# samukallio/path-tracer

Measured on AMD Instinct MI355X. Metric: Mrays/s + Msamples/s, Viking Room 1920x1080 1024spp, 1/2/4/8 GPUs, higher is better.
Workload: dtype f32; 1 GPU; C3 scene, one 1920x1080 1024-spp frame per step (Reset, Run(2), Run(1) until the frame's sample count reaches 1024 x pixels); each of 1 GPU(s) renders every pixel with its own RNG stream to 1/1 of the samples, then the reduce of radiance + sample counts to rank 0; spp_target=1024, streams=1, slots_per_launch_rank0=2073600, split=3, class_lists=False, frame_target_samples_rank0=2123366400, mesh_faces=3976, parallelism=sample-shards x1

## Files before the change

### include/pt_scene.h

```cpp
#ifndef PT_SCENE_H
#define PT_SCENE_H

#include <stdint.h>
#include "pt_packed.h"

#ifdef __cplusplus
extern "C" {
#endif

typedef struct pts_scene pts_scene;
typedef struct pts_entity pts_entity;
typedef struct pts_material pts_material;
typedef struct pts_texture pts_texture;
typedef struct pts_mesh pts_mesh;
typedef struct pts_prefab pts_prefab;

enum {
    PTS_ENTITY_ROOT = 0,
    PTS_ENTITY_CONTAINER = 1,
    PTS_ENTITY_CAMERA = 2,
    PTS_ENTITY_MESH_INSTANCE = 3,
    PTS_ENTITY_PLANE = 4,
    PTS_ENTITY_SPHERE = 5,
    PTS_ENTITY_CUBE = 6,
// ... 93 lines not shown
int  ptsSaveSpectrumTable(const char* path);
int  ptsLoadSpectrumTable(const char* path);
void ptsSetSpectrumTablePath(const char* path);

int  ptsDenoise(uint32_t width, uint32_t height, const float* accum_rgba, const pt_denoise_guide* guides,
                const pt_denoise_parameters* params, float* out_rgba);
int  ptsDenoisePair(uint32_t width, uint32_t height, const float* accum_a, const float* accum_b,
                    const pt_denoise_guide* guides, const pt_denoise_pair_parameters* params, float* out_rgba);

int  ptsReproject(uint32_t prev_width, uint32_t prev_height, const float* prev_accum,
                  const pt_denoise_guide* prev_guides, const pt_packed_camera* prev_camera, uint32_t width,
                  uint32_t height, const pt_denoise_guide* guides, const pt_packed_camera* camera,
                  const pt_reproject_parameters* params, float* out_rgba);
int  ptsShapeMotion(const pt_packed_shape* prev_shapes, uint32_t prev_count, const pt_packed_shape* shapes,
                    uint32_t count, pt_shape_motion* out);
int  ptsReprojectMoving(uint32_t prev_width, uint32_t prev_height, const float* prev_accum,
                        const pt_denoise_guide* prev_guides, const pt_packed_camera* prev_camera, uint32_t width,
                        uint32_t height, const pt_denoise_guide* guides, const pt_packed_camera* camera,
                        const pt_shape_motion* motion, uint32_t motion_count, const pt_reproject_parameters* params,
                        float* out_rgba);
int  ptsRectifyHistory(uint32_t width, uint32_t height, const float* history, const float* current,
                       const pt_denoise_guide* guides, const pt_rectify_parameters* params, float* out_rgba);
int  ptsDespike(uint32_t width, uint32_t height, const float* accum, const pt_denoise_guide* guides,
                const pt_despike_parameters* params, float* out_rgba);
int  ptsCentralCameraRay(const pt_packed_camera* camera, uint32_t x, uint32_t y, uint32_t width, uint32_t height,
                         float origin[3], float velocity[3]);
int  ptsAmbientOcclusionRays(const pt_ambient_occlusion_parameters* params, uint32_t x, uint32_t y,
                             const float origin[3], const float velocity[3], float time, const float normal[3],
                             float* out_origins, uint32_t* out_velocities, float* out_duration);
int  ptsGatherVisibilityRays(const pt_visibility_gather_parameters* params, uint32_t n, const float* points,
                             const float* normals, float* out_origins, uint32_t* out_velocities,
                             float* out_durations);
int  ptsGatherVisibilityReduce(uint32_t samples, uint32_t n, const uint32_t* packed, const uint64_t* occluded_bits,
                               pt_visibility_record* out);
uint32_t ptsVisibilitySkip(uint32_t state, uint32_t steps);
int  ptsSkyGatherRays(const pt_sky_gather_parameters* params, uint32_t n, const float* points, const float* normals,
                      float* out_origins, uint32_t* out_velocities, float* out_durations, float* out_lambda0);
int  ptsSkyGatherReduce(uint32_t samples, uint32_t n, const uint32_t* packed, const uint64_t* occluded_bits,
                        const float* contributions, pt_sky_record* out);
int  ptsSkyGatherBasis(uint32_t n, const uint32_t* packed, float* out);

int  ptsFrameStatistics(uint32_t width, uint32_t height, const float* accum_a, const float* accum_b,
                        pt_frame_statistics* out);
int  ptsTileStatistics(uint32_t width, uint32_t height, const float* accum_a, const float* accum_b,
                       float noise_threshold, pt_tile_statistics* out);
int    ptsStatsBin(float value);
double ptsStatsBinEdge(int bin);
int    ptsStatsPercentileBin(const uint32_t* histogram, double q);
double ptsStatsLogAverage(const uint32_t* histogram, double q_lo, double q_hi);
double ptsStatsAutoBrightness(const pt_frame_statistics* stats, double key, double q_lo, double q_hi);
double ptsStatsNoise(const pt_frame_statistics* stats, double q);
uint32_t ptsRayKey(const float origin[3], const float velocity[3], const float lo[3], const float hi[3]);

#ifdef __cplusplus
}
#endif

#endif
```

### path-tracer_amd/_native.py

```python
from __future__ import annotations

import ctypes as C
import os
from pathlib import Path

import numpy as np

PKG = Path(__file__).resolve().parent
SCENE_LIB_PATH = PKG / "libptscene.so"
HIP_LIB_PATH = PKG / "libpathtracer.so"


class NativeLibraryMissing(RuntimeError):
    pass



class pt_scene_packs(C.Structure):
    _fields_ = [
        ("globals", C.c_void_p),
        ("textures", C.c_void_p), ("texture_count", C.c_uint32),
        ("material_data", C.c_void_p), ("material_word_count", C.c_uint32),
        ("shapes", C.c_void_p), ("shape_count", C.c_uint32),
        ("shape_nodes", C.c_void_p), ("shape_node_count", C.c_uint32),
# ... 329 lines not shown
    "ptsDefaultLoadModelOptions": (None, [C.POINTER(pts_load_model_options)]),
    "ptsLoadTexture": (_vp, [_vp, C.c_char_p, _i32, C.c_char_p]),
    "ptsLoadImageRGBA8": (_i32, [C.c_char_p, C.POINTER(C.c_uint32), C.POINTER(C.c_uint32), _vp]),
    "ptsLoadModelAsPrefab": (_vp, [_vp, C.c_char_p, C.POINTER(pts_load_model_options)]),
    "ptsInstantiatePrefab": (_vp, [_vp, _vp, _vp]),
    "ptsLoadScene": (_vp, [C.c_char_p]),
    "ptsSaveScene": (_i32, [_vp, C.c_char_p]),
    "ptsSceneTextureCount": (_u32, [_vp]),
    "ptsSceneMaterialCount": (_u32, [_vp]),
    "ptsSceneMeshCount": (_u32, [_vp]),
    "ptsScenePrefabCount": (_u32, [_vp]),
    "ptsPrefabMeshCount": (_u32, [_vp]),
    "ptsPrefabMesh": (_vp, [_vp, _u32, C.POINTER(_vp), _fptr]),
    "ptsMeshVertexCount": (_u32, [_vp]),
    "ptsMeshFaceCount": (_u32, [_vp]),
    "ptsMeshVertices": (None, [_vp, _fptr]),
    "ptsMaterialType": (_i32, [_vp]),
    "ptsPackSceneData": (_u32, [_vp]),
    "ptsGetScenePacks": (None, [_vp, C.POINTER(pt_scene_packs)]),
    "ptsMarkDirty": (None, [_vp, _u32]),
    "ptsGetParametricSpectrumCoefficients": (_i32, [_fptr, _fptr]),
    "ptsBuildSpectrumTable": (_i32, [_i32]),
    "ptsSaveSpectrumTable": (_i32, [C.c_char_p]),
    "ptsLoadSpectrumTable": (_i32, [C.c_char_p]),
    "ptsSetSpectrumTablePath": (None, [C.c_char_p]),
    "ptsDenoise": (_i32, [_u32, _u32, _fptr, _vp, C.POINTER(pt_denoise_parameters), _fptr]),
    "ptsDenoisePair": (_i32, [_u32, _u32, _fptr, _fptr, _vp, C.POINTER(pt_denoise_pair_parameters), _fptr]),
    "ptsReproject": (_i32, [_u32, _u32, _fptr, _vp, C.POINTER(pt_packed_camera), _u32, _u32, _vp,
                            C.POINTER(pt_packed_camera), C.POINTER(pt_reproject_parameters), _fptr]),
    "ptsShapeMotion": (_i32, [_vp, _u32, _vp, _u32, _vp]),
    "ptsReprojectMoving": (_i32, [_u32, _u32, _fptr, _vp, C.POINTER(pt_packed_camera), _u32, _u32, _vp,
                                  C.POINTER(pt_packed_camera), _vp, _u32, C.POINTER(pt_reproject_parameters), _fptr]),
    "ptsRectifyHistory": (_i32, [_u32, _u32, _fptr, _fptr, _vp, C.POINTER(pt_rectify_parameters), _fptr]),
    "ptsDespike": (_i32, [_u32, _u32, _fptr, _vp, C.POINTER(pt_despike_parameters), _fptr]),
    "ptsCentralCameraRay": (_i32, [C.POINTER(pt_packed_camera), _u32, _u32, _u32, _u32, _fptr, _fptr]),
    "ptsAmbientOcclusionRays": (_i32, [C.POINTER(pt_ambient_occlusion_parameters), _u32, _u32, _fptr, _fptr, _f32,
                                       _fptr, _fptr, _u32ptr, _fptr]),
    "ptsGatherVisibilityRays": (_i32, [C.POINTER(pt_visibility_gather_parameters), _u32, _fptr, _fptr, _fptr, _u32ptr,
                                       _fptr]),
    "ptsGatherVisibilityReduce": (_i32, [_u32, _u32, _u32ptr, C.POINTER(C.c_uint64), _vp]),
    "ptsVisibilitySkip": (_u32, [_u32, _u32]),
    "ptsSkyGatherRays": (_i32, [C.POINTER(pt_sky_gather_parameters), _u32, _fptr, _fptr, _fptr, _u32ptr, _fptr, _fptr]),
    "ptsSkyGatherReduce": (_i32, [_u32, _u32, _u32ptr, C.POINTER(C.c_uint64), _fptr, _vp]),
    "ptsSkyGatherBasis": (_i32, [_u32, _u32ptr, _fptr]),
    "ptsFrameStatistics": (_i32, [_u32, _u32, _fptr, _fptr, C.POINTER(pt_frame_statistics)]),
    "ptsTileStatistics": (_i32, [_u32, _u32, _fptr, _fptr, _f32, _vp]),
    "ptsStatsBin": (_i32, [C.c_float]),
    "ptsStatsBinEdge": (C.c_double, [_i32]),
    "ptsStatsPercentileBin": (_i32, [_u32ptr, C.c_double]),
    "ptsStatsLogAverage": (C.c_double, [_u32ptr, C.c_double, C.c_double]),
    "ptsStatsAutoBrightness": (C.c_double, [C.POINTER(pt_frame_statistics), C.c_double, C.c_double, C.c_double]),
    "ptsStatsNoise": (C.c_double, [C.POINTER(pt_frame_statistics), C.c_double]),
    "ptsRayKey": (_u32, [_fptr, _fptr, _fptr, _fptr]),
}

HIP_API = {
    "ptGetLastError": (C.c_char_p, []),
    "ptGetDeviceCount": (_i32, [C.POINTER(_i32)]),
    "ptCreateDevice": (_vp, [_i32]),
    "ptDestroyDevice": (None, [_vp]),
    "ptSynchronize": (_i32, [_vp]),
    "ptCreateScene": (_vp, [_vp]),
    "ptUpdateScene": (_i32, [_vp, _vp, C.POINTER(pt_scene_packs), _u32]),
    "ptSetSceneStackFormat": (_i32, [_vp, _u32]),
    "ptSetSceneHitRecordForm": (_i32, [_vp, _u32]),
    "ptSetSceneExtendForm": (_i32, [_vp, _u32]),
    "ptGetSceneExtendForm": (_i32, [_vp, C.POINTER(C.c_uint32)]),
    "ptDestroyScene": (None, [_vp, _vp]),
    "ptCreateSampleBuffer": (_vp, [_vp, _u32, _u32]),
    "ptDestroySampleBuffer": (None, [_vp, _vp]),
    "ptReadSampleBuffer": (_i32, [_vp, _vp, _fptr]),
    "ptWriteSampleBuffer": (_i32, [_vp, _vp, _fptr]),
    "ptRenderSampleBuffer": (_i32, [_vp, _vp, C.POINTER(pt_resolve_parameters)]),
    "ptReadResolvedImage": (_i32, [_vp, _vp, _fptr]),
    "ptReadResolvedImageSRGB8": (_i32, [_vp, _vp, C.POINTER(C.c_uint8)]),
    "ptCreateBasicRenderer": (_vp, [_vp, _vp, _vp]),
    "ptCreateBasicRendererPartitioned": (_vp, [_vp, _vp, _vp, _u32, _u32]),
    "ptCreateBasicRendererStreams": (_vp, [_vp, _vp, _vp, _u32, _u32, _u32]),
    "ptMergeBasicRendererStreams": (_i32, [_vp, _vp]),
    "ptBasicRendererStreams": (_u32, [_vp]),
    "ptReadBasicRendererStreamState": (_i32, [_vp, _vp, _u32, _vp]),
    "ptWriteBasicRendererState": (_i32, [_vp, _vp, _vp]),
    "ptWriteBasicRendererStreamState": (_i32, [_vp, _vp, _u32, _vp]),
    "ptReadBasicRendererStreamAccumulator": (_i32, [_vp, _vp, _u32, _fptr]),
    "ptWriteBasicRendererStreamAccumulator": (_i32, [_vp, _vp, _u32, _fptr]),
    "ptGetBasicRendererShadeInfo": (_i32, [_vp, C.POINTER(pt_shade_info)]),
    "ptDestroyBasicRenderer": (None, [_vp, _vp]),
    "ptBasicRendererParams": (C.POINTER(pt_basic_renderer_params), [_vp]),
    "ptResetBasicRenderer": (_i32, [_vp, _vp]),
    "ptRunBasicRenderer": (_i32, [_vp, _vp, _u32]),
    "ptBasicRendererSlotCount": (_u32, [_vp]),
    "ptSetBasicRendererFusedRounds": (_i32, [_vp, _i32]),
    "ptRunBasicRendererRounds": (_i32, [_vp, _vp, _u32]),
    "ptSetBasicRendererRoundBatch": (_i32, [_vp, _u32]),
    "ptSetBasicRendererSplit": (_i32, [_vp, _u32]),
    "ptSetBasicRendererClassLists": (_i32, [_vp, _u32]),
    "ptGetBasicRendererClassLists": (_i32, [_vp, _u32ptr]),
    "ptGetBasicRendererSplit": (_i32, [_vp, _u32ptr, _u32ptr, _u32ptr]),
    "ptSetBasicRendererRayOrder": (_i32, [_vp, _u32]),
    "ptGetBasicRendererRayOrder": (_i32, [_vp, _u32ptr, _u32ptr]),
    "ptSetBasicRendererBlockMap": (_i32, [_vp, _u32]),
    "ptGetBasicRendererBlockMap": (_i32, [_vp, _u32ptr, _u32ptr]),
    "ptBlockMapGroupTileCount": (_u32, [_u32, _u32, _u32, _u32]),
    "ptBlockMapGroupTile": (_u32, [_u32, _u32, _u32, _u32, _u32]),
    "ptBlockMapGroupTileStart": (_u32, [_u32, _u32, _u32, _u32]),
    "ptBlockMapGroupUnitCount": (_u32, [_u32, _u32, _u32, _u32]),
# ... 119 lines not shown
```

### path-tracer_amd/csrc/hip/pt_device.hpp

```cpp
#pragma once

#include <hip/hip_runtime.h>
#include "../../../include/pt_glsl.h"
#include "../../../include/pt_packed.h"

#define PT_DEV __device__ __forceinline__

namespace ptd {

constexpr uint32_t SHAPE_INDEX_NONE = 0xFFFFFFFFu;
constexpr uint32_t TEXTURE_INDEX_NONE = 0xFFFFFFFFu;
constexpr uint32_t PT_SHAPE_FLAG_UV = 1u;

struct dscene {
    pt_packed_scene_globals g;
    const pt_packed_texture* textures;
    const uint32_t* material;
    const pt_packed_shape* shapes;
    const float4* shape_nodes;
    const float4* mesh_faces;
    const uint2* mesh_vertices;
    const float4* vertex_attr;
    const float* vertex_v;
    const float4* mesh_nodes;
    const pt_packed_camera* cameras;
    const float4* atlas;
    uint32_t atlas_w, atlas_h, atlas_layers;
    uint32_t atlas_tiled;
    uint32_t fast_div;
    uint32_t blas_words;
    uint32_t blas_firstbits;
    uint32_t stack16;
    uint32_t mat_classes;
    uint32_t vidx21;
    float vmf_inv_kappa, vmf_exp_m2k, vmf_norm;
    float sky_flat;
    uint32_t node_cache;
    uint32_t single_mesh;
    uint32_t mesh_root[2];
    float mesh_from[16];
};

#ifndef PT_NODE_CACHE_PAIRS
#define PT_NODE_CACHE_PAIRS 160
#endif

struct ray { pt3 Origin; pt3 Velocity; float Duration; };
struct medium { uint32_t Priority; pt4 IOR, AbsorptionRate, ScatteringRate; float ScatteringAnisotropy; };

PT_DEV pt3 xyz(float4 a) { return v3(a.x, a.y, a.z); }


PT_DEV pt3 TransformNormal(pt3 N, const float* From) { return normalize(vec_mul_mat4(N, From)); }
PT_DEV pt3 TransformDirection(pt3 D, const float* To) { return normalize(mat4_mul_vector(To, D)); }

PT_DEV pt3 SafeNormalize(pt3 V)
{
// ... 23 lines not shown
        float Sx = Px >= 0.0f ? 1.0f : -1.0f, Sy = Py >= 0.0f ? 1.0f : -1.0f;
        float Nx = (1.0f - pt_abs(Py)) * Sx;
        float Ny = (1.0f - pt_abs(Px)) * Sy;
        Px = Nx; Py = Ny;
    }
    return pt_pack_snorm16(Px) | (pt_pack_snorm16(Py) << 16);
}

PT_DEV pt3 UnpackUnitVector(uint32_t P)
{
    float Px = pt_unpack_snorm16(P & 0xFFFFu), Py = pt_unpack_snorm16(P >> 16);
    float Z = 1.0f - pt_abs(Px) - pt_abs(Py);
    if (Z < 0.0f) {
        float Sx = Px >= 0.0f ? 1.0f : -1.0f, Sy = Py >= 0.0f ? 1.0f : -1.0f;
        float Nx = (1.0f - pt_abs(Py)) * Sx;
        float Ny = (1.0f - pt_abs(Px)) * Sy;
        Px = Nx; Py = Ny;
    }
    return normalize(v3(Px, Py, Z));
}

PT_DEV float RecipForDiv(float b)
{
    float m = pt_abs(b);
    return (m >= 0x1p-100f && m <= 0x1p100f) ? 1.0f / b : pt_u2f(0x7fc00000u);
}

PT_DEV float XDiv(float a, float b, float y)
{
    float q = a * y;
    float r = __builtin_fmaf(-q, b, a);
    float q1 = __builtin_fmaf(r, y, q);
    float m = pt_abs(q1);
    if (!(m >= 0x1p-100f && m <= 0x1p100f && pt_abs(a) >= 0x1p-100f)) q1 = a / b;
    return q1;
}

PT_DEV float HwMin(float a, float b) { return __builtin_fminf(a, b); }
PT_DEV float HwMax(float a, float b) { return __builtin_fmaxf(a, b); }
PT_DEV float HwMin3(float a, float b, float c) { return __builtin_fminf(__builtin_fminf(a, b), c); }
PT_DEV float HwMax3(float a, float b, float c) { return __builtin_fmaxf(__builtin_fmaxf(a, b), c); }

PT_DEV float FastRcp(float d)
{
    float y = __builtin_amdgcn_rcpf(d);
    float e = __builtin_fmaf(-d, y, 1.0f);
    return __builtin_fmaf(e, y, y);
}


PT_DEV bool FastRcpRange(float d)
{
    float m = pt_abs(d);
    return (m >= 0x1p-126f) & (m < 0x1p126f);
}


PT_DEV bool FastDivRay(pt3 O, pt3 V)
{
    bool ok = true;
#define PT_CHECK_O(c) { float m = pt_abs(c); ok &= (m == 0.0f) | ((m >= 0x1p-50f) & (m <= 0x1p40f)); }
#define PT_CHECK_V(c) { float m = pt_abs(c); ok &= (m >= 0x1p-59f) & (m <= 0x1p27f); }
    PT_CHECK_O(O.x) PT_CHECK_O(O.y) PT_CHECK_O(O.z)
    PT_CHECK_V(V.x) PT_CHECK_V(V.y) PT_CHECK_V(V.z)
#undef PT_CHECK_O
#undef PT_CHECK_V
    return ok;
}

PT_DEV float FastQuot(float a, float b, float y)
{
    float q = a * y;
    float r = __builtin_fmaf(-q, b, a);
    return __builtin_fmaf(r, y, q);
}

PT_DEV float SlabEntry(float ax, float ay, float az, float bx, float by, float bz, float Reach)
{
    float EntryT = HwMax3(HwMin(ax, bx), HwMin(ay, by), HwMin(az, bz));
    float ExitT = HwMin3(HwMax(ax, bx), HwMax(ay, by), HwMax(az, bz));
    bool miss = (ExitT < EntryT) | (ExitT <= 0.0f) | (EntryT >= Reach);
    return miss ? PT_INFINITY : EntryT;
}

PT_DEV float IntersectBoundingBox(pt3 O, pt3 V, pt3 Y, float Reach, float4 MinAndX, float4 MaxAndX, bool exact)
{
    pt3 A = xyz(MinAndX) - O, B = xyz(MaxAndX) - O;
    if (exact)
        return SlabEntry(FastQuot(A.x, V.x, Y.x), FastQuot(A.y, V.y, Y.y), FastQuot(A.z, V.z, Y.z),
                         FastQuot(B.x, V.x, Y.x), FastQuot(B.y, V.y, Y.y), FastQuot(B.z, V.z, Y.z), Reach);
    return SlabEntry(A.x / V.x, A.y / V.y, A.z / V.z, B.x / V.x, B.y / V.y, B.z / V.z, Reach);
}

PT_DEV void IntersectBoxPair(pt3 O, pt3 V, pt3 Y, float Reach, float4 a0, float4 a1, float4 b0, float4 b1, bool exact,
                             float& TA, float& TB)
{
    if (exact) {
        TA = IntersectBoundingBox(O, V, Y, Reach, a0, a1, true);
        TB = IntersectBoundingBox(O, V, Y, Reach, b0, b1, true);
    } else {
        TA = IntersectBoundingBox(O, V, Y, Reach, a0, a1, false);
        TB = IntersectBoundingBox(O, V, Y, Reach, b0, b1, false);
    }
}

struct rng {
    uint32_t State;
// ... 287 lines not shown
```

### path-tracer_amd/csrc/hip/traverse.hpp

```cpp
#pragma once

#include "pt_device.hpp"

namespace ptd {

#define PT_LDS __attribute__((address_space(3)))
#define PT_GLOBAL __attribute__((address_space(1)))
typedef float f32x4 __attribute__((ext_vector_type(4)));
PT_DEV float4 F4(f32x4 v) { return make_float4(v.x, v.y, v.z, v.w); }



template <bool SPILL, int CAP, class E = uint32_t>
struct tstack {
    E* lds;
    uint32_t* spill;
    uint32_t stride;
    const float4* nc = nullptr;
    uint32_t ncn = 0;
    PT_DEV void put(uint32_t i, uint32_t v)
    {
        if (!SPILL || i < CAP) lds[i * 256] = (E)v;
        else spill[(i - CAP) * stride] = v;
    }
// ... 61 lines not shown
        L.HA = __float_as_uint(L.C.x);
        L.HB = 0;
    } else if (Type == PT_SHAPE_TYPE_SPHERE) {
        float Vv = dot(V, V);
        float P = dot(O, V);
        float Q = dot(O, O) - 1.0f;
        float D2 = P * P - Q * Vv;
        if (D2 < 0) return;
        float D = pt_sqrt(D2);
        if (D < P) return;
        float S0 = -P - D;
        float S1 = -P + D;
        float Sv = S0 < 0 ? S1 : S0;
        if (Sv < 0 || Sv > Vv * L.Time) return;
        L.Time = Sv / Vv;
        L.Shape = ShapeIndex;
        L.Prim = 0;
        L.C = O + V * L.Time;
        L.HA = __float_as_uint(L.C.x);
        L.HB = 0;
    } else if (Type == PT_SHAPE_TYPE_CUBE) {
        pt3 Mn = (v3s(-1) - O) / V;
        pt3 Mx = (v3s(+1) - O) / V;
        pt3 E = vmin(Mn, Mx);
        pt3 Lt = vmax(Mn, Mx);
        float T0 = pt_max(pt_max(E.x, E.y), E.z);
        float T1 = pt_min(pt_min(Lt.x, Lt.y), Lt.z);
        if (T1 < T0) return;
        if (T1 <= 0) return;
        float T = T0 < 0 ? T1 : T0;
        if (T >= L.Time) return;
        L.Time = T;
        L.Shape = ShapeIndex;
        L.Prim = 0;
        L.C = O + V * T;
        L.HA = __float_as_uint(L.C.x);
        L.HB = 0;
    }
}

PT_DEV void PackVertexIndices(uint32_t v0, uint32_t v1, uint32_t v2, uint32_t& A, uint32_t& B)
{
    A = v0 | (v1 << 21);
    B = (v1 >> 11) | (v2 << 10);
}

PT_DEV void UnpackVertexIndices(uint32_t A, uint32_t B, uint32_t& v0, uint32_t& v1, uint32_t& v2)
{
    v0 = A & 0x1FFFFFu;
    v1 = (A >> 21) | ((B & 0x3FFu) << 11);
    v2 = B >> 10;
}

PT_DEV bool FaceTest(const dscene& S, uint32_t F, const lane_state& L, bool valid, float& T, float& U, float& W,
                     uint32_t& VA, uint32_t& VB)
{
    uint32_t Fl = valid ? F : 0u;
    const float4* Fp = S.mesh_faces + 3 * (size_t)Fl;
    float4 a = Fp[0], b = Fp[1], c = Fp[2];
    pt3 P0 = xyz(a);
    pt3 Edge1 = xyz(b);
    pt3 Edge2 = xyz(c);
    PackVertexIndices(__float_as_uint(a.w), __float_as_uint(b.w), __float_as_uint(c.w), VA, VB);
    pt3 RCE2 = cross(L.V, Edge2);
    float Det = dot(Edge1, RCE2);
    float InvDet = 1.0f / Det;
    pt3 Sv = L.O - P0;
    U = InvDet * dot(Sv, RCE2);
    pt3 SCE1 = cross(Sv, Edge1);
    W = InvDet * dot(L.V, SCE1);
    T = InvDet * dot(Edge2, SCE1);
    return (pt_abs(Det) < PT_EPSILON) | (U < 0) | (U > 1) | (W < 0) | (U + W > 1) | (T < 0) | (T > L.Time) | !valid;
}

PT_DEV void LaneMeshFace(const dscene& S, uint32_t F, lane_state& L, bool valid = true)
{
    float T, U, W;
    uint32_t VA, VB;
    bool miss = FaceTest(S, F, L, valid, T, U, W, VA, VB);
    L.Time = miss ? L.Time : T;
    L.Shape = miss ? L.Shape : 0xFFFFFFFEu;
    L.Prim = miss ? L.Prim : F;
    L.HA = miss ? L.HA : VA;
    L.HB = miss ? L.HB : VB;
    L.C = v3(miss ? L.C.x : 1 - U - W, miss ? L.C.y : U, miss ? L.C.z : W);
}

struct no_stats {
    PT_DEV void face_step(bool) {}
    PT_DEV void coherence(uint32_t) {}
    PT_DEV void node(bool) {}
    PT_DEV void step() {}
    PT_DEV void internal() {}
    PT_DEV void leaf(uint32_t) {}
    PT_DEV void shape() {}
    PT_DEV void pop() {}
};
struct lane_stats {
    uint32_t steps = 0, internals = 0, leaves = 0, faces = 0, shapes = 0, pops = 0;
    uint32_t uniq[5] = {0, 0, 0, 0, 0};
    PT_DEV void coherence(uint32_t index)
    {
        uint64_t act = __ballot(1);
        uint32_t first = (uint32_t)__ffsll((long long)act) - 1u;
        uint32_t lane = __lane_id();
        uint32_t u = 0;
        bool done = false;
        for (;;) {
            uint64_t m = __ballot(!done);
            if (m == 0) break;
            uint32_t f = (uint32_t)__shfl(index, (int)(__ffsll((long long)m) - 1), 64);
            if (!done && index == f) done = true;
            u++;
        }
        if (lane == first) uniq[u == 1 ? 0 : u == 2 ? 1 : u <= 4 ? 2 : u <= 8 ? 3 : 4]++;
    }
    PT_DEV void node(bool) {}
    PT_DEV void step() { steps++; }
    PT_DEV void internal() { internals++; }
    PT_DEV void leaf(uint32_t n) { leaves++; faces += n; }
    PT_DEV void face_step(bool last) { faces++; leaves += last; }
    PT_DEV void shape() { shapes++; }
    PT_DEV void pop() { pops++; }
};

// ... 87 lines not shown
                uint32_t Root = Shape->MeshRootNodeIndex;
                SetLevelRay(S, L, O, V);
                L.blas = ShapeIndex;
                L.dB = 0;
                L.na = mesh_words[8 * Root + 3];
                L.nb = mesh_words[8 * Root + 7];
                return false;
            }
            IntersectAnalytic(Type, O, V, ShapeIndex, L);
        } else {
            ss.internal();
            uint32_t IA = Children & 0xFFFF, IB = Children >> 16;
            const float4* Ap = S.shape_nodes + 2 * (size_t)IA;
            const float4* Bp = S.shape_nodes + 2 * (size_t)IB;
            float4 a0 = Ap[0], a1 = Ap[1], b0 = Bp[0], b1 = Bp[1];
            float TA, TB;
            IntersectBoxPair(L.O, L.V, L.Y, L.Time, a0, a1, b0, b1, L.exact, TA, TB);
            bool goB = TA > TB;
            bool any = goB | (TA < PT_INFINITY);
            bool push = goB ? (TA < PT_INFINITY) : (TB < PT_INFINITY);
            if (push & (L.dT < 32)) st.put(L.dT++, goB ? IA : IB);
            if (any) {
                L.na = __float_as_uint(goB ? b0.w : a0.w);
                L.nb = __float_as_uint(goB ? b1.w : a1.w);
                return false;
            }
        }
    }
    if (L.dT > 0) {
        ss.pop();
        uint32_t I = st.get(--L.dT);
        L.na = shape_words[8 * I + 3];
        L.nb = shape_words[8 * I + 7];
        return false;
    }
    return true;
}

template <bool SPILL, int CAP, class Src, class Stats = no_stats, bool FACE_STEP = false, class SE = uint32_t>
PT_DEV bool LaneStep(const dscene& S, lane_state& L, tstack<SPILL, CAP, SE>& st, const Src& src, uint32_t slot,
                     Stats& ss)
{
    ss.step();
    bool tlas = L.blas == SHAPE_INDEX_NONE;
    if (FACE_STEP && !tlas) {
        const bool face = L.nb > 0;
        bool fmiss = true;
        float fT, fU, fW, TA, TB;
        uint32_t aw0, aw1, bw0, bw1, fVA, fVB;
        uint32_t pair = L.na;
        asm("" : "=v"(fT), "=v"(fU), "=v"(fW), "=v"(TA), "=v"(TB), "=v"(fVA), "=v"(fVB));
        asm("" : "=v"(aw0), "=v"(aw1), "=v"(bw0), "=v"(bw1));
        if (face) {
            fmiss = FaceTest(S, L.na, L, L.na < L.nb, fT, fU, fW, fVA, fVB);
            ss.face_step(L.na + 1 >= L.nb);
        } else {
            ss.node(true);
            ss.internal();
            ss.coherence(L.na);
            float4 a0, a1, b0, b1;
            if (L.na < st.ncn) {
                const PT_LDS f32x4* Cp = (const PT_LDS f32x4*)st.nc + 2 * L.na;
                a0 = F4(Cp[0]); a1 = F4(Cp[1]); b0 = F4(Cp[2]); b1 = F4(Cp[3]);
            } else {
                const PT_GLOBAL f32x4* Np = (const PT_GLOBAL f32x4*)S.mesh_nodes + 2 * (size_t)L.na;
                a0 = F4(Np[0]); a1 = F4(Np[1]); b0 = F4(Np[2]); b1 = F4(Np[3]);
            }
            IntersectBoxPair(L.O, L.V, L.Y, L.Time, a0, a1, b0, b1, L.exact, TA, TB);
            aw0 = __float_as_uint(a0.w), aw1 = __float_as_uint(a1.w);
            bw0 = __float_as_uint(b0.w), bw1 = __float_as_uint(b1.w);
        }
        L.Time = fmiss ? L.Time : fT;
        L.Shape = fmiss ? L.Shape : 0xFFFFFFFEu;
        L.Prim = fmiss ? L.Prim : L.na;
        L.HA = fmiss ? L.HA : fVA;
        L.HB = fmiss ? L.HB : fVB;
        L.C = v3(fmiss ? L.C.x : 1 - fU - fW, fmiss ? L.C.y : fU, fmiss ? L.C.z : fW);
        bool goB = TA > TB;
        float Tfar = goB ? TA : TB;
        bool push = !face & (Tfar < PT_INFINITY);
        bool moved = (face & (L.na + 1 < L.nb)) | (!face & (goB | (TA < PT_INFINITY)));
        if (push & (L.dB < 32)) {
            st.put(L.dT + L.dB++, BlasPush<SE>(S, goB ? aw0 : bw0, goB ? aw1 : bw1, pair + (goB ? 0u : 1u)));
        }
        uint32_t na = face ? L.na + 1 : (goB ? bw0 : aw0);
        uint32_t nb = face ? L.nb : (goB ? bw1 : aw1);
        if (!moved) {
            if (L.dB > 0) {
                ss.pop();
                BlasPop<SE>(S, st.get(L.dT + --L.dB), na, nb);
            } else {
                tlas = true;
            }
        }
        L.na = na;
        L.nb = nb;
        if (!tlas) return false;
        return TlasStep(S, L, st, src, slot, ss);
    }
    if (!tlas) {
        bool moved = false;
        if (L.nb > 0) {
            if (FACE_STEP) {
                LaneMeshFace(S, L.na, L, L.na < L.nb);
                bool last = ++L.na >= L.nb;
                ss.face_step(last);
                moved = !last;
            } else {
                ss.node(true);
                ss.leaf(L.nb - L.na);
                for (uint32_t F = L.na; F < L.nb; F++) LaneMeshFace(S, F, L);
            }
        } else {
            ss.node(true);
            ss.internal();
            uint32_t Index = L.na;
            ss.coherence(Index);
            const float4* Np = S.mesh_nodes + 2 * (size_t)Index;
            float4 a0 = Np[0], a1 = Np[1], b0 = Np[2], b1 = Np[3];
            float TA, TB;
            IntersectBoxPair(L.O, L.V, L.Y, L.Time, a0, a1, b0, b1, L.exact, TA, TB);
            bool goB = TA > TB;
            moved = goB | (TA < PT_INFINITY);
            bool push = goB ? (TA < PT_INFINITY) : (TB < PT_INFINITY);
            uint32_t aw0 = __float_as_uint(a0.w), aw1 = __float_as_uint(a1.w);
            uint32_t bw0 = __float_as_uint(b0.w), bw1 = __float_as_uint(b1.w);
            if (push & (L.dB < 32)) {
                st.put(L.dT + L.dB++, BlasPush<SE, !FACE_STEP>(S, goB ? aw0 : bw0, goB ? aw1 : bw1, Index + (goB ? 0u : 1u)));
            }
            if (moved) {
                L.na = goB ? bw0 : aw0;
                L.nb = goB ? bw1 : aw1;
            }
        }
        if (!moved) {
            if (L.dB > 0) {
                ss.pop();
                BlasPop<SE, !FACE_STEP>(S, st.get(L.dT + --L.dB), L.na, L.nb);
            } else {
                tlas = true;
            }
        }
    }
    if (!tlas) return false;
    return TlasStep(S, L, st, src, slot, ss);
}


PT_DEV void MeshBegin(const dscene& S, lane_state& L, pt3 O, pt3 V, float Duration)
{
    L.Time = Duration;
    L.Shape = SHAPE_INDEX_NONE;
    L.Prim = 0;
    L.C = v3s(0);
    L.HA = 0;
    L.HB = 0;
    L.dT = 0;
    L.dB = 0;
    L.blas = 0;
    SetLevelRay(S, L, mat4_mul_point(S.mesh_from, O), mat4_mul_vector(S.mesh_from, V));
    L.na = S.mesh_root[0];
    L.nb = S.mesh_root[1];
}

template <bool EXACT, bool SPILL, int CAP, class SE>
PT_DEV bool MeshStep(const dscene& S, lane_state& L, tstack<SPILL, CAP, SE>& st)
{
    const bool face = L.nb > 0;
    bool fmiss = true;
    float fT, fU, fW, TA, TB;
    uint32_t aw0, aw1, bw0, bw1, fVA, fVB;
    uint32_t pair = L.na;
    asm("" : "=v"(fT), "=v"(fU), "=v"(fW), "=v"(TA), "=v"(TB), "=v"(fVA), "=v"(fVB));
    asm("" : "=v"(aw0), "=v"(aw1), "=v"(bw0), "=v"(bw1));
    if (face) {
        fmiss = FaceTest(S, L.na, L, L.na < L.nb, fT, fU, fW, fVA, fVB);
    } else {
        float4 a0, a1, b0, b1;
        if (L.na < st.ncn) {
            const PT_LDS f32x4* Cp = (const PT_LDS f32x4*)st.nc + 2 * L.na;
            a0 = F4(Cp[0]); a1 = F4(Cp[1]); b0 = F4(Cp[2]); b1 = F4(Cp[3]);
        } else {
            const PT_GLOBAL f32x4* Np = (const PT_GLOBAL f32x4*)S.mesh_nodes + 2 * (size_t)L.na;
            a0 = F4(Np[0]); a1 = F4(Np[1]); b0 = F4(Np[2]); b1 = F4(Np[3]);
        }
        IntersectBoxPair(L.O, L.V, L.Y, L.Time, a0, a1, b0, b1, EXACT, TA, TB);
        aw0 = __float_as_uint(a0.w), aw1 = __float_as_uint(a1.w);
        bw0 = __float_as_uint(b0.w), bw1 = __float_as_uint(b1.w);
    }
    L.Time = fmiss ? L.Time : fT;
    L.Shape = fmiss ? L.Shape : 0xFFFFFFFEu;
    L.Prim = fmiss ? L.Prim : L.na;
    L.HA = fmiss ? L.HA : fVA;
    L.HB = fmiss ? L.HB : fVB;
    L.C = v3(fmiss ? L.C.x : 1 - fU - fW, fmiss ? L.C.y : fU, fmiss ? L.C.z : fW);
    bool goB = TA > TB;
    float Tfar = goB ? TA : TB;
    bool push = !face & (Tfar < PT_INFINITY);
    bool moved = (face & (L.na + 1 < L.nb)) | (!face & (goB | (TA < PT_INFINITY)));
    if (push & (L.dB < 32)) {
        st.put(L.dB++, BlasPush<SE>(S, goB ? aw0 : bw0, goB ? aw1 : bw1, pair + (goB ? 0u : 1u)));
    }
    uint32_t na = face ? L.na + 1 : (goB ? bw0 : aw0);
    uint32_t nb = face ? L.nb : (goB ? bw1 : aw1);
    const bool pop = !moved & (L.dB > 0);
    const bool done = !moved & (L.dB == 0);
    if (pop) BlasPop<SE>(S, st.get(--L.dB), na, nb);
    L.na = na;
    L.nb = nb;
    return done;
}

PT_DEV float4 CompactHit(const lane_state& Ln, bool vidx21)
{
    return make_float4(Ln.Time, __uint_as_float(Ln.Shape), __uint_as_float(vidx21 ? Ln.HA : Ln.Prim),
                       vidx21 ? __uint_as_float(Ln.HB) : Ln.C.x);
}

PT_DEV void HitAttributesV(const dscene& S, uint32_t ShapeIndex, bool packed, uint32_t Z, uint32_t Wd, pt3 C,
                           uint32_t& Material, pt3& Normal, pt3& TangentX, pt2& UV, bool uv_if_textured = false,
                           bool prims = true);

PT_DEV void HitAttributes(const dscene& S, uint32_t ShapeIndex, uint32_t Prim, pt3 C, uint32_t& Material, pt3& Normal,
                          pt3& TangentX, pt2& UV)
{
    HitAttributesV(S, ShapeIndex, false, Prim, 0u, C, Material, Normal, TangentX, UV);
}

PT_DEV void HitAttributesRecord(const dscene& S, uint32_t ShapeIndex, float4 h, float2 c, uint32_t& Material,
                                pt3& Normal, pt3& TangentX, pt2& UV, bool uv_if_textured = false, bool prims = true)
{
    const bool mesh = !prims || S.shapes[ShapeIndex].Type == PT_SHAPE_TYPE_MESH_INSTANCE;
    if (S.vidx21) {
        pt3 C = mesh ? v3(1 - c.x - c.y, c.x, c.y) : v3(h.z, c.x, c.y);
        HitAttributesV(S, ShapeIndex, true, __float_as_uint(h.z), __float_as_uint(h.w), C, Material, Normal, TangentX, UV,
                       uv_if_textured, prims);
    } else {
        HitAttributesV(S, ShapeIndex, false, __float_as_uint(h.z), 0u, v3(h.w, c.x, c.y), Material, Normal, TangentX, UV,
                       uv_if_textured, prims);
    }
}

PT_DEV void HitAttributesV(const dscene& S, uint32_t ShapeIndex, bool packed, uint32_t Z, uint32_t Wd, pt3 C,
                           uint32_t& Material, pt3& Normal, pt3& TangentX, pt2& UV, bool uv_if_textured, bool prims)
{
    UV = v2(0.0f, 0.0f);
    const pt_packed_shape* Shape = &S.shapes[ShapeIndex];
    Material = Shape->MaterialIndex;
    const bool uv = !uv_if_textured || (Shape->Pad0 & PT_SHAPE_FLAG_UV);
    int32_t Type = Shape->Type;
    const float* To = Shape->Transform.To;
    const float* From = Shape->Transform.From;
    const bool mesh = !prims || Type == PT_SHAPE_TYPE_MESH_INSTANCE;
    pt3 N, T = v3s(0.0f);
    if (mesh) {
        uint32_t i0, i1, i2;
        if (packed) {
            UnpackVertexIndices(Z, Wd, i0, i1, i2);
        } else {
// ... 47 lines not shown
```

### path-tracer_amd/csrc/scene/capi.cpp

```cpp
#include "scene.hpp"
#include "configs.hpp"
#include "image.hpp"
#include "../../../include/pt_scene.h"
#include "../../../include/pt_raykey.h"

#include <cstring>
#include <exception>
#include <new>
#include <string>
#include <vector>

using namespace pth;

namespace {
thread_local std::string g_err;
scene* S(pts_scene* s) { return reinterpret_cast<scene*>(s); }
entity* E(pts_entity* e) { return reinterpret_cast<entity*>(e); }
material* M(pts_material* m) { return reinterpret_cast<material*>(m); }
texture* T(pts_texture* t) { return reinterpret_cast<texture*>(t); }
mesh* Me(pts_mesh* m) { return reinterpret_cast<mesh*>(m); }

template <class R, class F>
R Guard(R fail, const char* what, F&& f)
{
    try {
        return f();
    } catch (const std::bad_alloc&) {
        g_err = std::string(what) + ": out of memory";
    } catch (const std::exception& e) {
        g_err = std::string(what) + ": " + e.what();
    } catch (...) {
        g_err = std::string(what) + ": unknown exception";
    }
    return fail;
}
}

extern "C" {

const char* ptsGetLastError(void) { return g_err.c_str(); }

pts_scene* ptsCreateScene(void) { return reinterpret_cast<pts_scene*>(CreateScene()); }
pts_scene* ptsCreateEmptyScene(void) { return reinterpret_cast<pts_scene*>(CreateEmptyScene()); }

pts_scene* ptsCreateConfigScene(int config, pts_config_info* info)
{
    config_info I{};
    scene* s = CreateConfigScene(config, &I);
    if (!s) { g_err = "unknown config " + std::to_string(config); return nullptr; }
    if (info) {
        info->width = I.width; info->height = I.height; info->spp = I.spp; info->camera_count = I.camera_count;
        info->render_flags = I.render_flags; info->termination_probability = I.termination_probability;
        info->mesh_face_count = I.mesh_face_count; info->shape_count = I.shape_count;
    }
    return reinterpret_cast<pts_scene*>(s);
}

// ... 301 lines not shown
int ptsMaterialType(pts_material* m) { return m ? (int)reinterpret_cast<material*>(m)->Type : -1; }

static entity* FindCamera(entity* e, uint32_t index)
{
    if (e->Type == ENTITY_TYPE_CAMERA && e->PackedCameraIndex == index) return e;
    for (entity* c : e->Children)
        if (entity* f = FindCamera(c, index)) return f;
    return nullptr;
}

pts_entity* ptsFindCamera(pts_scene* s, uint32_t packed_index)
{
    entity* e = FindCamera(&S(s)->Root, packed_index);
    if (!e) g_err = "no camera with packed index " + std::to_string(packed_index);
    return reinterpret_cast<pts_entity*>(e);
}

void ptsSetCameraTransform(pts_scene* s, pts_entity* c, const float p[3], const float r[3])
{
    if (p) E(c)->Transform.Position = vec3(p[0], p[1], p[2]);
    if (r) E(c)->Transform.Rotation = vec3(r[0], r[1], r[2]);
    S(s)->DirtyFlags |= PT_SCENE_DIRTY_CAMERAS;
}

uint32_t ptsPackSceneData(pts_scene* s) { return PackSceneData(S(s)); }
void ptsGetScenePacks(pts_scene* s, pt_scene_packs* out) { GetScenePacks(S(s), out); }
void ptsMarkDirty(pts_scene* s, uint32_t flags) { S(s)->DirtyFlags |= flags; }

int ptsGetParametricSpectrumCoefficients(const float rgb[3], float beta[3])
{
    vec3 b = GetParametricSpectrumCoefficients(GetSharedSpectrumTable(), vec3(rgb[0], rgb[1], rgb[2]));
    beta[0] = b.x; beta[1] = b.y; beta[2] = b.z;
    return 0;
}

int ptsBuildSpectrumTable(int threads)
{
    BuildParametricSpectrumTableForSRGB(GetSharedSpectrumTable(), threads);
    return 0;
}

int ptsSaveSpectrumTable(const char* path)
{
    return SaveParametricSpectrumTable(GetSharedSpectrumTable(), path) ? 0 : -1;
}

int ptsLoadSpectrumTable(const char* path)
{
    return LoadParametricSpectrumTable(GetSharedSpectrumTable(), path) ? 0 : -1;
}

void ptsSetSpectrumTablePath(const char* path) { SetSpectrumTablePath(path ? path : ""); }

uint32_t ptsRayKey(const float origin[3], const float velocity[3], const float lo[3], const float hi[3])
{
    if (!origin || !velocity || !lo || !hi) return 0xFFFFFFFFu;
    const pt_raykey_bounds B = pt_raykey_make_bounds(lo, hi);
    return pt_ray_key(origin[0], origin[1], origin[2], velocity[0], velocity[1], velocity[2], &B);
}

}
```

Measured before the change: 6676 Mrays/s.

## Use fast reciprocal in face test and wave-mask control flow in MeshStep

The ray-triangle test now uses a fast reciprocal and falls back to a true division only when some lane in the wave has a huge determinant. The miss predicate is merged into fewer min/max compares. Face and node addressing use 32-bit byte offsets when the stack entry type is 16-bit. MeshStep's branch logic is restructured around explicit wave ballot masks so the hit-update and node-push blocks are skipped when no lane needs them. A host-side reference face test is also added for checking. The fast reciprocal may differ slightly in precision from IEEE division, and the mask rewrite adds complexity to traversal control flow.

```diff
diff --git a/include/pt_facetest.h b/include/pt_facetest.h
--- /dev/null
+++ b/include/pt_facetest.h
@@ -0,0 +1,21 @@
+#ifndef PT_FACETEST_H
+#define PT_FACETEST_H
+
+#include "pt_fp.h"
+
+PT_HD int pt_face_miss(float Det, float U, float W, float T, float Time)
+{
+    const float lo = pt_min(pt_min(U, W), T);
+    const float hi = pt_max(U, U + W);
+    return (pt_abs(Det) < PT_EPSILON) | (lo < 0.0f) | (hi > 1.0f) | (T > Time);
+}
+
+#define PT_FAST_RCP_MIN 0x1p-126f
+#define PT_FAST_RCP_MAX 0x1p126f
+
+PT_HD int pt_face_needs_division(float Det)
+{
+    return !(pt_abs(Det) < PT_FAST_RCP_MAX);
+}
+
+#endif
diff --git a/include/pt_scene.h b/include/pt_scene.h
--- a/include/pt_scene.h
+++ b/include/pt_scene.h
@@ -169,6 +169,9 @@
 double ptsStatsNoise(const pt_frame_statistics* stats, double q);
 uint32_t ptsRayKey(const float origin[3], const float velocity[3], const float lo[3], const float hi[3]);
 
+int ptsFaceTest(uint32_t n, const float* det, const float* num_u, const float* num_w, const float* num_t,
+                const float* time, uint32_t* miss, float* u, float* w, float* t, uint32_t* divides);
+
 #ifdef __cplusplus
 }
 #endif
diff --git a/path-tracer_amd/_native.py b/path-tracer_amd/_native.py
--- a/path-tracer_amd/_native.py
+++ b/path-tracer_amd/_native.py
@@ -405,6 +405,7 @@
     "ptsStatsAutoBrightness": (C.c_double, [C.POINTER(pt_frame_statistics), C.c_double, C.c_double, C.c_double]),
     "ptsStatsNoise": (C.c_double, [C.POINTER(pt_frame_statistics), C.c_double]),
     "ptsRayKey": (_u32, [_fptr, _fptr, _fptr, _fptr]),
+    "ptsFaceTest": (_i32, [_u32, _fptr, _fptr, _fptr, _fptr, _fptr, _u32ptr, _fptr, _fptr, _fptr, _u32ptr]),
 }
 
 HIP_API = {
diff --git a/path-tracer_amd/csrc/hip/pt_device.hpp b/path-tracer_amd/csrc/hip/pt_device.hpp
--- a/path-tracer_amd/csrc/hip/pt_device.hpp
+++ b/path-tracer_amd/csrc/hip/pt_device.hpp
@@ -3,6 +3,7 @@
 #include <hip/hip_runtime.h>
 #include "../../../include/pt_glsl.h"
 #include "../../../include/pt_packed.h"
+#include "../../../include/pt_facetest.h"
 
 #define PT_DEV __device__ __forceinline__
 
@@ -132,7 +133,7 @@
 PT_DEV bool FastRcpRange(float d)
 {
     float m = pt_abs(d);
-    return (m >= 0x1p-126f) & (m < 0x1p126f);
+    return (m >= PT_FAST_RCP_MIN) & (m < PT_FAST_RCP_MAX);
 }
 
 
diff --git a/path-tracer_amd/csrc/hip/traverse.hpp b/path-tracer_amd/csrc/hip/traverse.hpp
--- a/path-tracer_amd/csrc/hip/traverse.hpp
+++ b/path-tracer_amd/csrc/hip/traverse.hpp
@@ -137,11 +137,13 @@
     v2 = B >> 10;
 }
 
+template <bool OFF32 = false>
 PT_DEV bool FaceTest(const dscene& S, uint32_t F, const lane_state& L, bool valid, float& T, float& U, float& W,
                      uint32_t& VA, uint32_t& VB)
 {
     uint32_t Fl = valid ? F : 0u;
-    const float4* Fp = S.mesh_faces + 3 * (size_t)Fl;
+    const float4* Fp = OFF32 ? (const float4*)((const char*)S.mesh_faces + __umul24(Fl, 48u))
+                             : S.mesh_faces + 3 * (size_t)Fl;
     float4 a = Fp[0], b = Fp[1], c = Fp[2];
     pt3 P0 = xyz(a);
     pt3 Edge1 = xyz(b);
@@ -149,13 +151,19 @@
     PackVertexIndices(__float_as_uint(a.w), __float_as_uint(b.w), __float_as_uint(c.w), VA, VB);
     pt3 RCE2 = cross(L.V, Edge2);
     float Det = dot(Edge1, RCE2);
-    float InvDet = 1.0f / Det;
+    float InvDet = FastRcp(Det);
+    const bool divide = pt_face_needs_division(Det);
+    if (__builtin_amdgcn_ballot_w64(divide) != 0) {
+        float d = Det;
+        asm volatile("" : "+v"(d));
+        if (divide) InvDet = 1.0f / d;
+    }
     pt3 Sv = L.O - P0;
     U = InvDet * dot(Sv, RCE2);
     pt3 SCE1 = cross(Sv, Edge1);
     W = InvDet * dot(L.V, SCE1);
     T = InvDet * dot(Edge2, SCE1);
-    return (pt_abs(Det) < PT_EPSILON) | (U < 0) | (U > 1) | (W < 0) | (U + W > 1) | (T < 0) | (T > L.Time) | !valid;
+    return (pt_face_miss(Det, U, W, T, L.Time) != 0) | !valid;
 }
 
 PT_DEV void LaneMeshFace(const dscene& S, uint32_t F, lane_state& L, bool valid = true)
@@ -349,7 +357,7 @@
         asm("" : "=v"(fT), "=v"(fU), "=v"(fW), "=v"(TA), "=v"(TB), "=v"(fVA), "=v"(fVB));
         asm("" : "=v"(aw0), "=v"(aw1), "=v"(bw0), "=v"(bw1));
         if (face) {
-            fmiss = FaceTest(S, L.na, L, L.na < L.nb, fT, fU, fW, fVA, fVB);
+            fmiss = FaceTest<sizeof(SE) == 2>(S, L.na, L, L.na < L.nb, fT, fU, fW, fVA, fVB);
             ss.face_step(L.na + 1 >= L.nb);
         } else {
             ss.node(true);
@@ -444,6 +452,14 @@
 }
 
 
+PT_DEV unsigned long long PtMaskNeU(uint32_t a, uint32_t b) { return __builtin_amdgcn_uicmp(a, b, 33); }
+PT_DEV unsigned long long PtMaskEqU(uint32_t a, uint32_t b) { return __builtin_amdgcn_uicmp(a, b, 32); }
+PT_DEV unsigned long long PtMaskLtU(uint32_t a, uint32_t b) { return __builtin_amdgcn_uicmp(a, b, 36); }
+PT_DEV unsigned long long PtMaskGtF(float a, float b) { return __builtin_amdgcn_fcmpf(a, b, 2); }
+PT_DEV unsigned long long PtMaskLtF(float a, float b) { return __builtin_amdgcn_fcmpf(a, b, 4); }
+PT_DEV unsigned long long PtActive() { return __builtin_amdgcn_ballot_w64(true); }
+PT_DEV bool PtLanes(unsigned long long m) { return __builtin_amdgcn_inverse_ballot_w64(m); }
+
 PT_DEV void MeshBegin(const dscene& S, lane_state& L, pt3 O, pt3 V, float Duration)
 {
     L.Time = Duration;
@@ -463,7 +479,8 @@
 template <bool EXACT, bool SPILL, int CAP, class SE>
 PT_DEV bool MeshStep(const dscene& S, lane_state& L, tstack<SPILL, CAP, SE>& st)
 {
-    const bool face = L.nb > 0;
+    const unsigned long long mF = PtMaskNeU(L.nb, 0u);
+    const bool face = PtLanes(mF);
     bool fmiss = true;
     float fT, fU, fW, TA, TB;
     uint32_t aw0, aw1, bw0, bw1, fVA, fVB;
@@ -471,10 +488,19 @@
     asm("" : "=v"(fT), "=v"(fU), "=v"(fW), "=v"(TA), "=v"(TB), "=v"(fVA), "=v"(fVB));
     asm("" : "=v"(aw0), "=v"(aw1), "=v"(bw0), "=v"(bw1));
     if (face) {
-        fmiss = FaceTest(S, L.na, L, L.na < L.nb, fT, fU, fW, fVA, fVB);
+        fmiss = FaceTest<sizeof(SE) == 2>(S, L.na, L, L.na < L.nb, fT, fU, fW, fVA, fVB);
     } else {
         float4 a0, a1, b0, b1;
-        if (L.na < st.ncn) {
+        if (sizeof(SE) == 2) {
+            const uint32_t off = L.na * 32u;
+            if (L.na < st.ncn) {
+                const PT_LDS f32x4* Cp = (const PT_LDS f32x4*)((const PT_LDS char*)st.nc + off);
+                a0 = F4(Cp[0]); a1 = F4(Cp[1]); b0 = F4(Cp[2]); b1 = F4(Cp[3]);
+            } else {
+                const PT_GLOBAL f32x4* Np = (const PT_GLOBAL f32x4*)((const PT_GLOBAL char*)S.mesh_nodes + off);
+                a0 = F4(Np[0]); a1 = F4(Np[1]); b0 = F4(Np[2]); b1 = F4(Np[3]);
+            }
+        } else if (L.na < st.ncn) {
             const PT_LDS f32x4* Cp = (const PT_LDS f32x4*)st.nc + 2 * L.na;
             a0 = F4(Cp[0]); a1 = F4(Cp[1]); b0 = F4(Cp[2]); b1 = F4(Cp[3]);
         } else {
@@ -485,23 +511,32 @@
         aw0 = __float_as_uint(a0.w), aw1 = __float_as_uint(a1.w);
         bw0 = __float_as_uint(b0.w), bw1 = __float_as_uint(b1.w);
     }
-    L.Time = fmiss ? L.Time : fT;
-    L.Shape = fmiss ? L.Shape : 0xFFFFFFFEu;
-    L.Prim = fmiss ? L.Prim : L.na;
-    L.HA = fmiss ? L.HA : fVA;
-    L.HB = fmiss ? L.HB : fVB;
-    L.C = v3(fmiss ? L.C.x : 1 - fU - fW, fmiss ? L.C.y : fU, fmiss ? L.C.z : fW);
-    bool goB = TA > TB;
-    float Tfar = goB ? TA : TB;
-    bool push = !face & (Tfar < PT_INFINITY);
-    bool moved = (face & (L.na + 1 < L.nb)) | (!face & (goB | (TA < PT_INFINITY)));
-    if (push & (L.dB < 32)) {
-        st.put(L.dB++, BlasPush<SE>(S, goB ? aw0 : bw0, goB ? aw1 : bw1, pair + (goB ? 0u : 1u)));
-    }
-    uint32_t na = face ? L.na + 1 : (goB ? bw0 : aw0);
-    uint32_t nb = face ? L.nb : (goB ? bw1 : aw1);
-    const bool pop = !moved & (L.dB > 0);
-    const bool done = !moved & (L.dB == 0);
+    const bool anyF = mF != 0, anyI = (PtActive() & ~mF) != 0;
+    if (anyF) {
+        L.Time = fmiss ? L.Time : fT;
+        L.Shape = fmiss ? L.Shape : 0xFFFFFFFEu;
+        L.Prim = fmiss ? L.Prim : L.na;
+        L.HA = fmiss ? L.HA : fVA;
+        L.HB = fmiss ? L.HB : fVB;
+        L.C = v3(fmiss ? L.C.x : 1 - fU - fW, fmiss ? L.C.y : fU, fmiss ? L.C.z : fW);
+    }
+    uint32_t na = L.na + 1;
+    uint32_t nb = L.nb;
+    unsigned long long mMoved = mF & PtMaskLtU(na, nb);
+    if (anyI) {
+        const unsigned long long mB = PtMaskGtF(TA, TB);
+        const bool goB = PtLanes(mB);
+        const float Tfar = goB ? TA : TB;
+        mMoved |= ~mF & (mB | PtMaskLtF(TA, PT_INFINITY));
+        if (PtLanes(~mF & PtMaskLtF(Tfar, PT_INFINITY) & PtMaskLtU(L.dB, 32u))) {
+            st.put(L.dB++, BlasPush<SE>(S, goB ? aw0 : bw0, goB ? aw1 : bw1, pair + (goB ? 0u : 1u)));
+        }
+        na = face ? na : (goB ? bw0 : aw0);
+        nb = face ? nb : (goB ? bw1 : aw1);
+    }
+    const unsigned long long mEmpty = PtMaskEqU(L.dB, 0u);
+    const bool pop = PtLanes(~mMoved & ~mEmpty & PtActive());
+    const bool done = PtLanes(~mMoved & mEmpty);
     if (pop) BlasPop<SE>(S, st.get(--L.dB), na, nb);
     L.na = na;
     L.nb = nb;
diff --git a/path-tracer_amd/csrc/scene/capi.cpp b/path-tracer_amd/csrc/scene/capi.cpp
--- a/path-tracer_amd/csrc/scene/capi.cpp
+++ b/path-tracer_amd/csrc/scene/capi.cpp
@@ -3,6 +3,7 @@
 #include "image.hpp"
 #include "../../../include/pt_scene.h"
 #include "../../../include/pt_raykey.h"
+#include "../../../include/pt_facetest.h"
 
 #include <cstring>
 #include <exception>
@@ -410,6 +411,28 @@
 
 void ptsSetSpectrumTablePath(const char* path) { SetSpectrumTablePath(path ? path : ""); }
 
+int ptsFaceTest(uint32_t n, const float* det, const float* num_u, const float* num_w, const float* num_t,
+                const float* time, uint32_t* miss, float* u, float* w, float* t, uint32_t* divides)
+{
+    if (!det || !num_u || !num_w || !num_t || !time || !miss || !u || !w || !t || !divides) return -1;
+    for (uint32_t i = 0; i < n; i++) {
+        const float d = det[i];
+        float inv;
+        divides[i] = (uint32_t)pt_face_needs_division(d);
+        if (divides[i]) {
+            inv = 1.0f / d;
+        } else {
+            const float y = 1.0f / d;
+            inv = pt_fma(pt_fma(-d, y, 1.0f), y, y);
+        }
+        u[i] = inv * num_u[i];
+        w[i] = inv * num_w[i];
+        t[i] = inv * num_t[i];
+        miss[i] = (uint32_t)pt_face_miss(d, u[i], w[i], t[i], time[i]);
+    }
+    return 0;
+}
+
 uint32_t ptsRayKey(const float origin[3], const float velocity[3], const float lo[3], const float hi[3])
 {
     if (!origin || !velocity || !lo || !hi) return 0xFFFFFFFFu;
```

New measurement: 7128 Mrays/s (median of 6 runs). 6.8% higher.
